# pashtari/factorizer

Measured on AMD Instinct MI355X. Metric: volumes/sec fwd+bwd, Swin Factorizer 128^3, higher is better.
Workload: dtype f32

## Files before the change

### factorizer_amd/csrc/conv3.hip

```cpp
#include "gemm_bx.h"

namespace fz {

template <typename AT>
struct Conv3ArgsT {
  const AT* x;
  const float* w;
  const float* bias;
  AT* y;
  int B, Cin, M, D, H, W;
  BlockPrologueArgs pro;
};

template <int MB, typename AT>
__global__ __launch_bounds__(256, 2) void conv3_fwd_kernel(Conv3ArgsT<AT> p) {
  extern __shared__ __attribute__((aligned(16))) float As[];
  const int lane = threadIdx.x & 63, wave = threadIdx.x >> 6;
  const int j = lane & 31, h = lane >> 5;
  const int64_t V = (int64_t)p.D * p.H * p.W;
  const int tiles_per_sample = (int)((V + 511) / 512);
  const int b = blockIdx.x / tiles_per_sample;
  const int64_t n0 = ((int64_t)(blockIdx.x % tiles_per_sample) * 4 + wave) * 128;
  const int m0 = blockIdx.y * 32 * MB;
  const int ncp = p.Cin / 2;
  const int nA = ncp * 27;

  for (int base = threadIdx.x; base < nA * MB * 64; base += blockDim.x * 8) {
    float tmp[8];
#pragma unroll
    for (int uu = 0; uu < 8; ++uu) {
      const int idx = base + uu * blockDim.x;
      const bool in = idx < nA * MB * 64;
      const int ii = in ? idx : 0;
      const int l = ii & 63, mb = (ii >> 6) % MB, a = ii / (64 * MB);
      const int m = m0 + mb * 32 + (l & 31);
      const int c = 2 * (a / 27) + (l >> 5), tap = a % 27;
      const int mc = m < p.M ? m : p.M - 1;
      const float wv = p.w[((int64_t)mc * p.Cin + c) * 27 + tap];
      tmp[uu] = (in && m < p.M) ? wv : 0.f;
    }
#pragma unroll
    for (int uu = 0; uu < 8; ++uu) {
      const int idx = base + uu * blockDim.x;
      if (idx < nA * MB * 64) As[idx] = tmp[uu];
    }
  }
  __syncthreads();

  const int64_t col = n0 + 4 * j;
  const bool col_ok = col < V;
  const int64_t cc = col_ok ? col : 0;
  const int w0 = (int)(cc % p.W);
  const int h0 = (int)((cc / p.W) % p.H);
  const int d0 = (int)(cc / ((int64_t)p.W * p.H));
  const bool lok = w0 > 0, rok = w0 + 4 < p.W;

  f32x16 acc[MB][4];
#pragma unroll
  for (int mb = 0; mb < MB; ++mb)
#pragma unroll
    for (int q = 0; q < 4; ++q)
#pragma unroll
      for (int r = 0; r < 16; ++r) acc[mb][q][r] = 0.f;

  for (int cp = 0; cp < ncp; ++cp) {
    const AT* plane = p.x + ((int64_t)b * p.Cin + 2 * cp + h) * V;
#pragma unroll
    for (int kd = 0; kd < 3; ++kd) {
#pragma unroll
      for (int kh = 0; kh < 3; ++kh) {
        const int zd = d0 + kd - 1, zh = h0 + kh - 1;
        const bool ok = col_ok && zd >= 0 && zd < p.D && zh >= 0 && zh < p.H;
        const int zdc = zd < 0 ? 0 : (zd >= p.D ? p.D - 1 : zd);
        const int zhc = zh < 0 ? 0 : (zh >= p.H ? p.H - 1 : zh);
        const AT* row = plane + ((int64_t)zdc * p.H + zhc) * p.W;
        const float4 t = ld4(row + w0);
        const float lf = aget(row + (lok ? w0 - 1 : w0));
        const float rt = aget(row + (rok ? w0 + 4 : w0));
        const float c0 = ok ? t.x : 0.f, c1 = ok ? t.y : 0.f, c2 = ok ? t.z : 0.f, c3 = ok ? t.w : 0.f;
        const float l0 = (ok && lok) ? lf : 0.f, r0 = (ok && rok) ? rt : 0.f;
        const float bv[3][4] = {{l0, c0, c1, c2}, {c0, c1, c2, c3}, {c1, c2, c3, r0}};
#pragma unroll
        for (int kw = 0; kw < 3; ++kw) {
          const int a = cp * 27 + (kd * 3 + kh) * 3 + kw;
#pragma unroll
          for (int mb = 0; mb < MB; ++mb) {
            const float av = As[(a * MB + mb) * 64 + lane];
#pragma unroll
            for (int q = 0; q < 4; ++q)
              acc[mb][q] = __builtin_amdgcn_mfma_f32_32x32x2f32(av, bv[kw][q], acc[mb][q], 0, 0, 0);
          }
        }
      }
    }
  }
  if (!col_ok) return;
#pragma unroll
  for (int mb = 0; mb < MB; ++mb)
#pragma unroll
    for (int r = 0; r < 16; ++r) {
      const int m = m0 + mb * 32 + (r & 3) + 8 * (r >> 2) + 4 * h;
      if (m >= p.M) continue;
      const float bs = p.bias ? p.bias[m] : 0.f;
      st4(p.y + ((int64_t)b * p.M + m) * V + col,
          make_float4(acc[mb][0][r] + bs, acc[mb][1][r] + bs, acc[mb][2][r] + bs, acc[mb][3][r] + bs));
    }
}

template <int MB, int CP, typename AT, bool PRO = false>
__global__ __launch_bounds__(256, 2) void conv3_fwd_bx_kernel(Conv3ArgsT<AT> p) {
  static_assert(!PRO || MB == 1, "the block prologue needs all 32 output channels in one row block");
  constexpr int NTA = BxTerms<AT>::A, NTB = bx_terms_b<AT>(BXPRO_NONE);
  constexpr int NS = CP * 27;
  constexpr int NG = (NS + 7) / 8;
  __shared__ __attribute__((aligned(16))) __bf16 As[NG * MB * NTA * 64 * 8];
  __shared__ float sBias[32 * MB];
  __shared__ __attribute__((aligned(16))) __bf16 Apro[PRO ? 2 * 3 * 64 * 8 : 8];
  __shared__ float twp[PRO ? 32 : 1];
  if constexpr (PRO) ln_inproj_stage(Apro, twp, p.pro, (int)threadIdx.x, 256);
  const int lane = threadIdx.x & 63, wave = threadIdx.x >> 6;
  const int j = lane & 31, h = lane >> 5;
  const int64_t V = (int64_t)p.D * p.H * p.W;
  const int tiles_per_sample = (int)((V + 511) / 512);
  const int b = blockIdx.x / tiles_per_sample;
  const int64_t n0 = ((int64_t)(blockIdx.x % tiles_per_sample) * 4 + wave) * 128;
  const int m0 = blockIdx.y * 32 * MB;
  const int Cin = 2 * CP;

  for (int idx = threadIdx.x; idx < NG * MB * 64; idx += 256) {
    const int l = idx & 63, mb = (idx >> 6) % MB, g = idx / (64 * MB);
    const int m = m0 + mb * 32 + (l & 31);
    const int mc = m < p.M ? m : p.M - 1;
    float wv[8];
#pragma unroll
    for (int e = 0; e < 8; ++e) {
      const int a = 8 * g + e;
      const int ac = a < NS ? a : NS - 1;
      const int c = 2 * (ac / 27) + (l >> 5), tap = ac % 27;
      const float t = p.w[((int64_t)mc * Cin + c) * 27 + tap];
      wv[e] = (a < NS && m < p.M) ? t : 0.f;
    }
    bx8 t3[NTA];
    bx_split<NTA>(wv, t3);
#pragma unroll
    for (int i = 0; i < NTA; ++i) *reinterpret_cast<bx8*>(&As[(((g * MB + mb) * NTA + i) * 64 + l) * 8]) = t3[i];
  }
  if (threadIdx.x < 32 * MB) {
    const int m = m0 + threadIdx.x;
    sBias[threadIdx.x] = (p.bias != nullptr && m < p.M) ? p.bias[m] : 0.f;
  }
  __syncthreads();

  const int64_t col = n0 + 4 * j;
  const bool col_ok = col < V;
  const int64_t cc = col_ok ? col : 0;
  const int w0 = (int)(cc % p.W);
  const int h0 = (int)((cc / p.W) % p.H);
  const int d0 = (int)(cc / ((int64_t)p.W * p.H));
  const bool lok = w0 > 0, rok = w0 + 4 < p.W;

  f32x16 acc[MB][4];
#pragma unroll
  for (int mb = 0; mb < MB; ++mb)
#pragma unroll
    for (int q = 0; q < 4; ++q)
#pragma unroll
      for (int r = 0; r < 16; ++r) acc[mb][q][r] = 0.f;

  float xg[4][8];
#pragma unroll
  for (int cp = 0; cp < CP; ++cp) {
    const AT* plane = p.x + ((int64_t)b * Cin + 2 * cp + h) * V;
#pragma unroll
    for (int kd = 0; kd < 3; ++kd) {
#pragma unroll
      for (int kh = 0; kh < 3; ++kh) {
        const int zd = d0 + kd - 1, zh = h0 + kh - 1;
        const bool ok = col_ok && zd >= 0 && zd < p.D && zh >= 0 && zh < p.H;
        const int zdc = zd < 0 ? 0 : (zd >= p.D ? p.D - 1 : zd);
        const int zhc = zh < 0 ? 0 : (zh >= p.H ? p.H - 1 : zh);
        const AT* row = plane + ((int64_t)zdc * p.H + zhc) * p.W;
        const float4 t = ld4(row + w0);
        const float lf = aget(row + (lok ? w0 - 1 : w0));
        const float rt = aget(row + (rok ? w0 + 4 : w0));
        const float c0 = ok ? t.x : 0.f, c1 = ok ? t.y : 0.f, c2 = ok ? t.z : 0.f, c3 = ok ? t.w : 0.f;
        const float l0 = (ok && lok) ? lf : 0.f, r0 = (ok && rok) ? rt : 0.f;
        const float bv[3][4] = {{l0, c0, c1, c2}, {c0, c1, c2, c3}, {c1, c2, c3, r0}};
#pragma unroll
        for (int kw = 0; kw < 3; ++kw) {
          const int a = cp * 27 + (kd * 3 + kh) * 3 + kw;
#pragma unroll
          for (int q = 0; q < 4; ++q) xg[q][a & 7] = bv[kw][q];
          if ((a & 7) == 7 || a == NS - 1) {
            const int g = a >> 3;
            if (a == NS - 1) {
#pragma unroll
              for (int e = (NS - 1) % 8 + 1; e < 8; ++e)
#pragma unroll
                for (int q = 0; q < 4; ++q) xg[q][e] = 0.f;
            }
            bx8 bop[4][NTB];
#pragma unroll
            for (int q = 0; q < 4; ++q) bx_split<NTB>(xg[q], bop[q]);
#pragma unroll
            for (int mb = 0; mb < MB; ++mb) {
              bx8 aop[NTA];
#pragma unroll
              for (int i = 0; i < NTA; ++i)
                aop[i] = *reinterpret_cast<const bx8*>(&As[(((g * MB + mb) * NTA + i) * 64 + lane) * 8]);
#pragma unroll
              for (int q = 0; q < 4; ++q) bx_mfma<NTA, NTB>(acc[mb][q], aop, bop[q]);
            }
          }
        }
      }
    }
  }
  if (!col_ok) return;
  float yv[PRO ? 4 : 1][16];
#pragma unroll
  for (int mb = 0; mb < MB; ++mb)
#pragma unroll
    for (int r = 0; r < 16; ++r) {
      const int rl = (r & 3) + 8 * (r >> 2) + 4 * h;
      const int m = m0 + mb * 32 + rl;
      const float bs = sBias[mb * 32 + rl];
      const float4 o = make_float4(acc[mb][0][r] + bs, acc[mb][1][r] + bs, acc[mb][2][r] + bs, acc[mb][3][r] + bs);
      if (m < p.M) st4(p.y + ((int64_t)b * p.M + m) * V + col, o);
      if constexpr (PRO) {
        constexpr bool R = sizeof(AT) == 2;
        yv[0][r] = R ? (float)(AT)o.x : o.x; yv[1][r] = R ? (float)(AT)o.y : o.y;
        yv[2][r] = R ? (float)(AT)o.z : o.z; yv[3][r] = R ? (float)(AT)o.w : o.w;
      }
    }
  if constexpr (PRO) {
    float mu[4], rs[4];
    f32x16 tacc[4];
    ln_inproj_tile<4>(yv, Apro, p.pro.ln_eps, lane, mu, rs, tacc);
    AT* tb = reinterpret_cast<AT*>(p.pro.t) + (int64_t)b * 32 * V + col;
#pragma unroll
    for (int r = 0; r < 16; ++r) {
      const int rl = (r & 3) + 8 * (r >> 2) + 4 * h;
      const float add = twp[rl];
      st4(tb + (int64_t)rl * V, make_float4(fmaxf(tacc[0][r] + add, 0.f), fmaxf(tacc[1][r] + add, 0.f), fmaxf(tacc[2][r] + add, 0.f),
                                            fmaxf(tacc[3][r] + add, 0.f)));
    }
    if (h == 0) {
      float* so = p.pro.stats + (int64_t)b * 2 * V + col;
      *reinterpret_cast<float4*>(so) = make_float4(mu[0], mu[1], mu[2], mu[3]);
      *reinterpret_cast<float4*>(so + V) = make_float4(rs[0], rs[1], rs[2], rs[3]);
    }
  }
}

template <typename AT>
struct Conv3WgradArgsT {
  const AT* gy;
  const AT* x;
  float* part;
  float* part_bias;
  int B, Cin, M, D, H, W;
  int tiles_per_unit;
};

constexpr int kXs = 44;

template <int KB, typename AT, bool BX = false>
__global__ __launch_bounds__(256) void conv3_wgrad_kernel(Conv3WgradArgsT<AT> a) {
  extern __shared__ __attribute__((aligned(16))) float lds[];
  const int lane = threadIdx.x & 63, wave = threadIdx.x >> 6;
  const int nrow = a.Cin * 9;
  const int per_wave = 32 * 36 + 36 * kXs;
  float* Pt = lds + wave * per_wave;
  float* Xs = Pt + 32 * 36;
  const int K = 27 * a.Cin;
  const int m0 = blockIdx.y * 32;
  const int64_t V = (int64_t)a.D * a.H * a.W;
  const int64_t tiles_per_sample = V / 32;
  const int64_t total = tiles_per_sample * a.B;
  const int64_t unit = (int64_t)blockIdx.x * 4 + wave;
  const int64_t t_begin = unit * a.tiles_per_unit, t_end = min(t_begin + a.tiles_per_unit, total);
  const int c = lane & 31, h = lane >> 5;

  int xoff[KB];
#pragma unroll
  for (int jb = 0; jb < KB; ++jb) {
    const int k = jb * 32 + c;
    const int kc = k < K ? k : 0;
    const int ci = kc / 27, tap = kc % 27;
    xoff[jb] = (ci * 9 + tap / 3) * kXs + 3 + (tap % 3);
  }
  f32x16 acc[KB];
#pragma unroll
  for (int jb = 0; jb < KB; ++jb)
#pragma unroll
    for (int r = 0; r < 16; ++r) acc[jb][r] = 0.f;
  float psum = 0.f;

  float4 pv[4], hv[5];
  float ev[2];
  int tb, td, th, tw;
  {
    const unsigned tps32 = (unsigned)tiles_per_sample;
    const unsigned t0 = (unsigned)__builtin_amdgcn_readfirstlane((int)t_begin);
    const unsigned rem = t0 % tps32, row = rem / (unsigned)(a.W / 32);
    tb = (int)(t0 / tps32);
    tw = (int)(rem % (unsigned)(a.W / 32)) * 32;
    th = (int)(row % (unsigned)a.H);
    td = (int)(row / (unsigned)a.H);
  }
  const unsigned bias = (unsigned)((a.H + 1) * a.W + 1);
  unsigned goff[4], xo[5], eo[2];
  unsigned xsafe[5], esafe[2];
  unsigned mask = 0;
  bool gvalid[4];
#pragma unroll
  for (int i = 0; i < 4; ++i) {
    const int m = m0 + (lane >> 3) + 8 * i;
    gvalid[i] = m < a.M;
    goff[i] = (unsigned)((m < a.M ? m : a.M - 1) * V + (lane & 7) * 4);
  }
  auto tap_bits = [&](int kd, int kh) { return (unsigned)((kd == 0) | ((kd == 2) << 1) | ((kh == 0) << 2) | ((kh == 2) << 3)); };
#pragma unroll
  for (int i = 0; i < 5; ++i) {
    const int q = lane + 64 * i;
    const int rr = min(q >> 3, nrow - 1), cq = q & 7;
    const int ci = rr / 9, kd = (rr % 9) / 3, kh = rr % 3;
    xo[i] = (unsigned)(ci * V + ((kd - 1) * a.H + (kh - 1)) * a.W + cq * 4 + (int64_t)bias);
    xsafe[i] = (unsigned)(ci * V + cq * 4 + (int64_t)bias);
    mask |= tap_bits(kd, kh) << (4 * i);
  }
#pragma unroll
  for (int i = 0; i < 2; ++i) {
    const int id = lane + 64 * i;
    const int rr = min(id >> 1, nrow - 1), side = id & 1;
    const int ci = rr / 9, kd = (rr % 9) / 3, kh = rr % 3;
    eo[i] = (unsigned)(ci * V + ((kd - 1) * a.H + (kh - 1)) * a.W + (side ? 32 : -1) + (int64_t)bias);
    esafe[i] = (unsigned)(ci * V + (int64_t)bias);
  }
  unsigned emask = 0, enever = 0;
#pragma unroll
  for (int i = 0; i < 2; ++i) {
    const int id = lane + 64 * i;
    const int rr = min(id >> 1, nrow - 1), side = id & 1;
    const int kd = (rr % 9) / 3, kh = rr % 3;
    emask |= (tap_bits(kd, kh) | (side ? 0x20u : 0x10u)) << (8 * i);
    enever |= ((id >> 1) < nrow ? 0u : 1u) << i;
  }
  unsigned xnever = 0;
#pragma unroll
  for (int i = 0; i < 5; ++i) xnever |= (((lane + 64 * i) >> 3) < nrow ? 0u : 1u) << i;
  auto issue = [&]() {
    const int b = tb, w0 = tw, h0 = th, d0 = td;
    const unsigned f4 = (unsigned)((d0 == 0) | ((d0 == a.D - 1) << 1) | ((h0 == 0) << 2) | ((h0 == a.H - 1) << 3));
    const unsigned f20 = f4 * 0x11111u;
    const unsigned fe = (f4 | ((w0 == 0) << 4) | ((w0 + 32 == a.W) << 5)) * 0x101u;
    const int64_t n0 = ((int64_t)d0 * a.H + h0) * a.W + w0;
    const AT* gbase = a.gy + (int64_t)b * a.M * V + n0;
    const AT* xbase = a.x + (int64_t)b * a.Cin * V + n0 - (int64_t)bias;
    tw += 32;
    if (tw == a.W) { tw = 0; if (++th == a.H) { th = 0; if (++td == a.D) { td = 0; ++tb; } } }
    const unsigned bad = mask & f20, ebad = emask & fe;
#pragma unroll
    for (int i = 0; i < 4; ++i) {
      const float4 v = ld4(gbase + goff[i]);
      pv[i] = gvalid[i] ? v : make_float4(0.f, 0.f, 0.f, 0.f);
    }
#pragma unroll
    for (int i = 0; i < 5; ++i) {
      const bool ok = ((bad >> (4 * i)) & 0xfu) == 0 && ((xnever >> i) & 1u) == 0;
      const float4 v = ld4(xbase + (ok ? xo[i] : xsafe[i]));
      hv[i] = ok ? v : make_float4(0.f, 0.f, 0.f, 0.f);
    }
#pragma unroll
    for (int i = 0; i < 2; ++i) {
      const bool ok = ((ebad >> (8 * i)) & 0x3fu) == 0 && ((enever >> i) & 1u) == 0;
      const float v = aget(xbase + (ok ? eo[i] : esafe[i]));
      ev[i] = ok ? v : 0.f;
    }
  };

  if (t_begin < t_end) issue();
  for (int64_t t = t_begin; t < t_end; ++t) {
#pragma unroll
    for (int i = 0; i < 4; ++i)
      *reinterpret_cast<float4*>(Pt + ((lane >> 3) + 8 * i) * 36 + (lane & 7) * 4) = pv[i];
#pragma unroll
    for (int i = 0; i < 5; ++i) {
      const int q = lane + 64 * i;
      if (q < 288) *reinterpret_cast<float4*>(Xs + (q >> 3) * kXs + 4 + (q & 7) * 4) = hv[i];
    }
#pragma unroll
    for (int i = 0; i < 2; ++i) {
      const int id = lane + 64 * i;
      if (id < 72) Xs[(id >> 1) * kXs + ((id & 1) ? 36 : 3)] = ev[i];
    }
    __builtin_amdgcn_fence(__ATOMIC_ACQ_REL, "wavefront");
    if (t + 1 < t_end) issue();
    if constexpr (BX) {
      constexpr int NTA = BxTerms<AT>::A;
      constexpr int NT = sizeof(AT) == 4 ? 3 : 1;
      (void)NTA;
#pragma unroll
      for (int g = 0; g < 2; ++g) {
        float a8[8];
        const float4 a0 = *reinterpret_cast<const float4*>(Pt + c * 36 + 16 * g + 8 * h);
        const float4 a1 = *reinterpret_cast<const float4*>(Pt + c * 36 + 16 * g + 8 * h + 4);
        a8[0] = a0.x; a8[1] = a0.y; a8[2] = a0.z; a8[3] = a0.w; a8[4] = a1.x; a8[5] = a1.y; a8[6] = a1.z; a8[7] = a1.w;
        psum += ((a8[0] + a8[1]) + (a8[2] + a8[3])) + ((a8[4] + a8[5]) + (a8[6] + a8[7]));
        bx8 aop[NT];
        bx_split<NT>(a8, aop);
#pragma unroll
        for (int jb = 0; jb < KB; ++jb) {
          float b8[8];
#pragma unroll
          for (int e = 0; e < 8; ++e) b8[e] = Xs[xoff[jb] + 16 * g + 8 * h + e];
          bx8 bop[NT];
          bx_split<NT>(b8, bop);
          bx_mfma<NT, NT>(acc[jb], aop, bop);
        }
      }
    } else {
#pragma unroll 4
    for (int s = 0; s < 16; ++s) {
      const float av = Pt[c * 36 + 2 * s + h];
      psum += av;
#pragma unroll
      for (int jb = 0; jb < KB; ++jb) {
        const float bv = Xs[xoff[jb] + 2 * s + h];
        acc[jb] = __builtin_amdgcn_mfma_f32_32x32x2f32(av, bv, acc[jb], 0, 0, 0);
      }
    }
    }
    __builtin_amdgcn_fence(__ATOMIC_ACQ_REL, "wavefront");
  }

  __syncthreads();
  float* red = lds;
#pragma unroll
  for (int jb = 0; jb < KB; ++jb) {
#pragma unroll
    for (int r = 0; r < 16; ++r) {
      const int row = (r & 3) + 8 * (r >> 2) + 4 * h;
      red[wave * 1024 + row * 32 + c] = acc[jb][r];
    }
    __syncthreads();
    for (int e = threadIdx.x; e < 1024; e += 256) {
      const float sres = (red[e] + red[1024 + e]) + (red[2048 + e] + red[3072 + e]);
      const int m = m0 + (e >> 5), k = jb * 32 + (e & 31);
      if (m < a.M && k < K) a.part[((int64_t)blockIdx.x * a.M + m) * K + k] = sres;
    }
    __syncthreads();
  }
  {
    const float sres = psum + __shfl_xor(psum, 32, 64);
    if (h == 0) red[wave * 32 + c] = sres;
    __syncthreads();
    if (threadIdx.x < 32) {
      const int m = m0 + threadIdx.x;
      if (m < a.M)
        a.part_bias[(int64_t)blockIdx.x * a.M + m] =
            (red[threadIdx.x] + red[32 + threadIdx.x]) + (red[64 + threadIdx.x] + red[96 + threadIdx.x]);
    }
  }
}

}

using namespace fz;

template <typename AT>
static int conv3_fwd_launch(const void* x, const float* w, const float* bias, void* y, int B, int Cin, int M, int D,
                            int H, int W, int products, const fz_block_prologue* pro, fz_stream_t stream) {
  Conv3ArgsT<AT> p{(const AT*)x, w, bias, (AT*)y, B, Cin, M, D, H, W, BlockPrologueArgs{}};
  if (pro) {
    if (!(Cin == 4 && M == 32 && products_split(products)))
      return fail(FZ_E_UNSUPPORTED, "fz_conv3_fwd2: the block prologue needs C_in = 4, 32 output channels, split-bf16 products (fz_conv3_prologue_supported)");
    p.pro = BlockPrologueArgs{pro->ln_g, pro->ln_b, pro->ln_eps, pro->w, pro->t, pro->stats};
  }
  const int64_t V = (int64_t)D * H * W;
  const int mblocks = (M + 31) / 32;
  const int MB = mblocks >= 2 ? 2 : 1;
  const size_t lds = (size_t)(Cin / 2) * 27 * MB * 64 * sizeof(float);
  if (lds > 65536) return fail(FZ_E_UNSUPPORTED, "fz_conv3_fwd: C_in too large for the stem kernel");
  dim3 grid((unsigned)(((V + 511) / 512) * B), (unsigned)((mblocks + MB - 1) / MB)), block(256);
  hipStream_t st = (hipStream_t)stream;
  if (Cin == 4 && products_split(products)) {
    if (MB == 2) hipLaunchKernelGGL((conv3_fwd_bx_kernel<2, 2, AT>), grid, block, 0, st, p);
    else if (pro) hipLaunchKernelGGL((conv3_fwd_bx_kernel<1, 2, AT, true>), grid, block, 0, st, p);
    else hipLaunchKernelGGL((conv3_fwd_bx_kernel<1, 2, AT>), grid, block, 0, st, p);
    FZ_LAUNCH_CHECK();
    return FZ_OK;
  }
  if (MB == 2) hipLaunchKernelGGL((conv3_fwd_kernel<2, AT>), grid, block, lds, st, p);
  else hipLaunchKernelGGL((conv3_fwd_kernel<1, AT>), grid, block, lds, st, p);
  FZ_LAUNCH_CHECK();
  return FZ_OK;
}

extern "C" int fz_conv3_prologue_supported(int Cin, int M, int W, int products) {
  return (Cin == 4 && M == 32 && W >= 4 && (W & 3) == 0 && products_split(products)) ? 1 : 0;
}

extern "C" int fz_conv3_fwd2(const void* x, const float* w, const float* bias, void* y, int B, int Cin, int M, int D,
                             int H, int W, int act_dtype, int products, const fz_block_prologue* pro, fz_stream_t stream) {
  if (!x || !w || !y) return fail(FZ_E_ARG, "fz_conv3_fwd: null pointer");
  if (pro && (!pro->ln_g || !pro->ln_b || !pro->w || !pro->t || !pro->stats)) return fail(FZ_E_ARG, "fz_conv3_fwd2: incomplete block prologue");
  if (B < 0 || Cin < 2 || (Cin & 1) || M < 1 || D < 1 || H < 1 || W < 4 || (W & 3))
    return fail(FZ_E_UNSUPPORTED, "fz_conv3_fwd: needs even C_in and W % 4 == 0");
  if (B == 0) return FZ_OK;
  if (act_dtype == FZ_STORE_F32) return conv3_fwd_launch<float>(x, w, bias, y, B, Cin, M, D, H, W, products, pro, stream);
  if (act_dtype == FZ_STORE_BF16) return conv3_fwd_launch<bf16>(x, w, bias, y, B, Cin, M, D, H, W, products, pro, stream);
  return fail(FZ_E_ARG, "fz_conv3_fwd: bad act_dtype");
}

extern "C" int fz_conv3_fwd(const void* x, const float* w, const float* bias, void* y, int B, int Cin, int M, int D,
                            int H, int W, int act_dtype, int products, fz_stream_t stream) {
  return fz_conv3_fwd2(x, w, bias, y, B, Cin, M, D, H, W, act_dtype, products, nullptr, stream);
}

static int conv3_units(int64_t total_tiles, int* tiles_per_unit) {
  int64_t units_target = 4096;
  int64_t tpu = (total_tiles + units_target - 1) / units_target;
  if (tpu < 1) tpu = 1;
  *tiles_per_unit = (int)tpu;
  const int64_t units = (total_tiles + tpu - 1) / tpu;
  return (int)((units + 3) / 4);
}

extern "C" int fz_conv3_wgrad_chunks(int B, int D, int H, int W) {
  int tpu;
  return conv3_units(((int64_t)D * H * W / 32) * B, &tpu);
}

template <typename AT>
static int conv3_wgrad_launch(const void* gy, const void* x, float* part, float* part_bias, int B, int Cin,
                              int M, int D, int H, int W, int products, fz_stream_t stream) {
  Conv3WgradArgsT<AT> a{(const AT*)gy, (const AT*)x, part, part_bias, B, Cin, M, D, H, W, 1};
  const int nchunk = conv3_units(((int64_t)D * H * W / 32) * B, &a.tiles_per_unit);
  const size_t lds = (size_t)4 * (32 * 36 + 36 * kXs) * sizeof(float);
  const size_t lds_red = 4096 * sizeof(float);
  dim3 grid(nchunk, (M + 31) / 32), block(256);
  if (products_split(products))
    hipLaunchKernelGGL((conv3_wgrad_kernel<4, AT, true>), grid, block, lds > lds_red ? lds : lds_red, (hipStream_t)stream, a);
  else
    hipLaunchKernelGGL((conv3_wgrad_kernel<4, AT, false>), grid, block, lds > lds_red ? lds : lds_red, (hipStream_t)stream, a);
  FZ_LAUNCH_CHECK();
  return FZ_OK;
}

extern "C" int fz_conv3_wgrad_partials(const void* gy, const void* x, float* part, float* part_bias, int B, int Cin,
                                       int M, int D, int H, int W, int act_dtype, int products, fz_stream_t stream) {
  if (!gy || !x || !part || !part_bias) return fail(FZ_E_ARG, "fz_conv3_wgrad: null pointer");
  if (B < 1 || Cin < 1 || M < 1 || (W % 32) || 27 * Cin > 128 || Cin * 9 > 36)
    return fail(FZ_E_UNSUPPORTED, "fz_conv3_wgrad: needs W % 32 == 0 and C_in <= 4");
  {
    const int64_t V = (int64_t)D * H * W;
    if ((V / 32) * B >= ((int64_t)1 << 31) || (int64_t)(M < 32 ? 32 : M) * V >= ((int64_t)1 << 32) ||
        (int64_t)Cin * V + (int64_t)(H + 1) * W + 64 >= ((int64_t)1 << 32))
      return fail(FZ_E_UNSUPPORTED, "fz_conv3_wgrad: volume too large for the kernel's 32-bit offsets");
  }
  if (act_dtype == FZ_STORE_F32) return conv3_wgrad_launch<float>(gy, x, part, part_bias, B, Cin, M, D, H, W, products, stream);
  if (act_dtype == FZ_STORE_BF16) return conv3_wgrad_launch<bf16>(gy, x, part, part_bias, B, Cin, M, D, H, W, products, stream);
  return fail(FZ_E_ARG, "fz_conv3_wgrad: bad act_dtype");
}
```

Baseline: 130.9.

## Pre-split bf16 operands once in conv3 fwd and wgrad, remap wgrad blocks per XCD

In the stem conv forward kernel, the row values are now split into bf16 terms once per (kd,kh) and packed as bf16 pairs, instead of being re-split per 8-element group. Address math moves to 32-bit offsets with boundary flag masks, and out-of-range columns stay in the loop with guarded stores. In wgrad, when the multi-term bf16 path is in use, the input tile is pre-split into bf16 levels stored in LDS and read back with alignbit shifts, avoiding repeated per-jb splitting. Blocks are also remapped so contiguous units land on the same XCD. This adds a 32-bit volume limit check and more LDS per wave.

Measured after the change: 130.9. Within noise of the previous version (-0.0%).

```diff
diff --git a/factorizer_amd/csrc/conv3.hip b/factorizer_amd/csrc/conv3.hip
--- a/factorizer_amd/csrc/conv3.hip
+++ b/factorizer_amd/csrc/conv3.hip
@@ -1,6 +1,8 @@
 #include "gemm_bx.h"
 
 namespace fz {
+
+typedef unsigned u32x4 __attribute__((ext_vector_type(4)));
 
 template <typename AT>
 struct Conv3ArgsT {
@@ -153,11 +155,17 @@
 
   const int64_t col = n0 + 4 * j;
   const bool col_ok = col < V;
-  const int64_t cc = col_ok ? col : 0;
-  const int w0 = (int)(cc % p.W);
-  const int h0 = (int)((cc / p.W) % p.H);
-  const int d0 = (int)(cc / ((int64_t)p.W * p.H));
+  const unsigned cc = col_ok ? (unsigned)col : 0u;
+  const unsigned rowi = cc / (unsigned)p.W;
+  const int w0 = (int)(cc % (unsigned)p.W);
+  const int h0 = (int)(rowi % (unsigned)p.H);
+  const int d0 = (int)(rowi / (unsigned)p.H);
   const bool lok = w0 > 0, rok = w0 + 4 < p.W;
+  const unsigned flags = (unsigned)((d0 == 0) | ((d0 == p.D - 1) << 1) | ((h0 == 0) << 2) | ((h0 == p.H - 1) << 3) | ((col_ok ? 0 : 1) << 4));
+  const unsigned Vu = (unsigned)V, HW = (unsigned)p.H * (unsigned)p.W, Wu = (unsigned)p.W;
+  const AT* xb = p.x + (int64_t)b * Cin * V;
+  const unsigned lo_c = (unsigned)h * Vu + cc;
+  const unsigned lo_l = lok ? lo_c - 1u : lo_c, lo_r = rok ? lo_c + 4u : lo_c;
 
   f32x16 acc[MB][4];
 #pragma unroll
@@ -167,41 +175,69 @@
 #pragma unroll
       for (int r = 0; r < 16; ++r) acc[mb][q][r] = 0.f;
 
-  float xg[4][8];
+  unsigned bw[4][NTB][4];
+  float pend[4][NTB];
 #pragma unroll
   for (int cp = 0; cp < CP; ++cp) {
-    const AT* plane = p.x + ((int64_t)b * Cin + 2 * cp + h) * V;
+    const unsigned cbase = (unsigned)(2 * cp) * Vu;
 #pragma unroll
     for (int kd = 0; kd < 3; ++kd) {
 #pragma unroll
       for (int kh = 0; kh < 3; ++kh) {
-        const int zd = d0 + kd - 1, zh = h0 + kh - 1;
-        const bool ok = col_ok && zd >= 0 && zd < p.D && zh >= 0 && zh < p.H;
-        const int zdc = zd < 0 ? 0 : (zd >= p.D ? p.D - 1 : zd);
-        const int zhc = zh < 0 ? 0 : (zh >= p.H ? p.H - 1 : zh);
-        const AT* row = plane + ((int64_t)zdc * p.H + zhc) * p.W;
-        const float4 t = ld4(row + w0);
-        const float lf = aget(row + (lok ? w0 - 1 : w0));
-        const float rt = aget(row + (rok ? w0 + 4 : w0));
-        const float c0 = ok ? t.x : 0.f, c1 = ok ? t.y : 0.f, c2 = ok ? t.z : 0.f, c3 = ok ? t.w : 0.f;
-        const float l0 = (ok && lok) ? lf : 0.f, r0 = (ok && rok) ? rt : 0.f;
-        const float bv[3][4] = {{l0, c0, c1, c2}, {c0, c1, c2, c3}, {c1, c2, c3, r0}};
+        constexpr unsigned kColBit = 0x10u;
+        const unsigned tb = (unsigned)((kd == 0) | ((kd == 2) << 1) | ((kh == 0) << 2) | ((kh == 2) << 3)) | kColBit;
+        const bool ok = (flags & tb) == 0;
+        const unsigned goff = ok ? cbase + (unsigned)(kd - 1) * HW + (unsigned)(kh - 1) * Wu : cbase;
+        const float4 t = ld4(xb + (lo_c + goff));
+        const float lf = aget(xb + (lo_l + goff));
+        const float rt = aget(xb + (lo_r + goff));
+        float rv[NTB][6];
+        rv[0][0] = (ok && lok) ? lf : 0.f; rv[0][1] = ok ? t.x : 0.f; rv[0][2] = ok ? t.y : 0.f;
+        rv[0][3] = ok ? t.z : 0.f; rv[0][4] = ok ? t.w : 0.f; rv[0][5] = (ok && rok) ? rt : 0.f;
+#pragma unroll
+        for (int l = 1; l < NTB; ++l)
+#pragma unroll
+          for (int i = 0; i < 6; i += 2) {
+            const fx2 v = {rv[l - 1][i], rv[l - 1][i + 1]};
+            const fx2 d = v - __builtin_convertvector(__builtin_convertvector(v, bx2), fx2);
+            rv[l][i] = d[0]; rv[l][i + 1] = d[1];
+          }
 #pragma unroll
         for (int kw = 0; kw < 3; ++kw) {
           const int a = cp * 27 + (kd * 3 + kh) * 3 + kw;
 #pragma unroll
-          for (int q = 0; q < 4; ++q) xg[q][a & 7] = bv[kw][q];
+          for (int q = 0; q < 4; ++q)
+#pragma unroll
+            for (int l = 0; l < NTB; ++l) {
+              if ((a & 1) == 0) {
+                pend[q][l] = rv[l][kw + q];
+                if (a == NS - 1) {
+                  const fx2 v = {pend[q][l], 0.f};
+                  bw[q][l][(a & 7) >> 1] = __builtin_bit_cast(unsigned, __builtin_convertvector(v, bx2));
+                }
+              } else {
+                const fx2 v = {pend[q][l], rv[l][kw + q]};
+                bw[q][l][(a & 7) >> 1] = __builtin_bit_cast(unsigned, __builtin_convertvector(v, bx2));
+              }
+            }
           if ((a & 7) == 7 || a == NS - 1) {
             const int g = a >> 3;
             if (a == NS - 1) {
 #pragma unroll
-              for (int e = (NS - 1) % 8 + 1; e < 8; ++e)
-#pragma unroll
-                for (int q = 0; q < 4; ++q) xg[q][e] = 0.f;
+              for (int e = ((NS - 1) % 8) / 2 + 1; e < 4; ++e)
+#pragma unroll
+                for (int q = 0; q < 4; ++q)
+#pragma unroll
+                  for (int l = 0; l < NTB; ++l) bw[q][l][e] = 0u;
             }
             bx8 bop[4][NTB];
 #pragma unroll
-            for (int q = 0; q < 4; ++q) bx_split<NTB>(xg[q], bop[q]);
+            for (int q = 0; q < 4; ++q)
+#pragma unroll
+              for (int l = 0; l < NTB; ++l) {
+                const u32x4 o = {bw[q][l][0], bw[q][l][1], bw[q][l][2], bw[q][l][3]};
+                bop[q][l] = __builtin_bit_cast(bx8, o);
+              }
 #pragma unroll
             for (int mb = 0; mb < MB; ++mb) {
               bx8 aop[NTA];
@@ -216,7 +252,7 @@
       }
     }
   }
-  if (!col_ok) return;
+  if constexpr (!PRO) { if (!col_ok) return; }
   float yv[PRO ? 4 : 1][16];
 #pragma unroll
   for (int mb = 0; mb < MB; ++mb)
@@ -226,7 +262,7 @@
       const int m = m0 + mb * 32 + rl;
       const float bs = sBias[mb * 32 + rl];
       const float4 o = make_float4(acc[mb][0][r] + bs, acc[mb][1][r] + bs, acc[mb][2][r] + bs, acc[mb][3][r] + bs);
-      if (m < p.M) st4(p.y + ((int64_t)b * p.M + m) * V + col, o);
+      if (m < p.M && col_ok) st4(p.y + ((int64_t)b * p.M + m) * V + col, o);
       if constexpr (PRO) {
         constexpr bool R = sizeof(AT) == 2;
         yv[0][r] = R ? (float)(AT)o.x : o.x; yv[1][r] = R ? (float)(AT)o.y : o.y;
@@ -242,10 +278,11 @@
     for (int r = 0; r < 16; ++r) {
       const int rl = (r & 3) + 8 * (r >> 2) + 4 * h;
       const float add = twp[rl];
-      st4(tb + (int64_t)rl * V, make_float4(fmaxf(tacc[0][r] + add, 0.f), fmaxf(tacc[1][r] + add, 0.f), fmaxf(tacc[2][r] + add, 0.f),
-                                            fmaxf(tacc[3][r] + add, 0.f)));
-    }
-    if (h == 0) {
+      if (col_ok)
+        st4(tb + (int64_t)rl * V, make_float4(fmaxf(tacc[0][r] + add, 0.f), fmaxf(tacc[1][r] + add, 0.f), fmaxf(tacc[2][r] + add, 0.f),
+                                              fmaxf(tacc[3][r] + add, 0.f)));
+    }
+    if (h == 0 && col_ok) {
       float* so = p.pro.stats + (int64_t)b * 2 * V + col;
       *reinterpret_cast<float4*>(so) = make_float4(mu[0], mu[1], mu[2], mu[3]);
       *reinterpret_cast<float4*>(so + V) = make_float4(rs[0], rs[1], rs[2], rs[3]);
@@ -265,30 +302,71 @@
 
 constexpr int kXs = 44;
 
+constexpr int kXl = 18;
+constexpr int kXr = 3 * kXl;
+constexpr int conv3_wgrad_per_wave(bool lv) { return 32 * 36 + 36 * (lv ? kXr : kXs); }
+constexpr bool conv3_wgrad_levels(int nt) { return nt == 3; }
+template <typename AT> struct Conv3WgradTerms { static constexpr int N = sizeof(AT) == 4 ? 3 : 1; };
+
+template <int NT>
+__device__ __forceinline__ void bx_split2(float x0, float x1, unsigned (&t)[NT]) {
+  fx2 v = {x0, x1};
+  const bx2 a = __builtin_convertvector(v, bx2);
+  t[0] = __builtin_bit_cast(unsigned, a);
+  if constexpr (NT >= 2) {
+    v = v - __builtin_convertvector(a, fx2);
+    const bx2 b = __builtin_convertvector(v, bx2);
+    t[1] = __builtin_bit_cast(unsigned, b);
+    if constexpr (NT >= 3) {
+      v = v - __builtin_convertvector(b, fx2);
+      const bx2 c = __builtin_convertvector(v, bx2);
+      t[2] = __builtin_bit_cast(unsigned, c);
+    }
+  }
+}
+
+__device__ __forceinline__ int conv3_wgrad_logical_block() {
+  const int nb = (int)gridDim.x, bid = (int)blockIdx.x;
+  if (nb < 16) return bid;
+  const int q = nb / 8, r = nb % 8, xcd = bid % 8, i = bid / 8;
+  return (xcd < r ? xcd * (q + 1) : r * (q + 1) + (xcd - r) * q) + i;
+}
+
 template <int KB, typename AT, bool BX = false>
 __global__ __launch_bounds__(256) void conv3_wgrad_kernel(Conv3WgradArgsT<AT> a) {
   extern __shared__ __attribute__((aligned(16))) float lds[];
   const int lane = threadIdx.x & 63, wave = threadIdx.x >> 6;
   const int nrow = a.Cin * 9;
-  const int per_wave = 32 * 36 + 36 * kXs;
-  float* Pt = lds + wave * per_wave;
-  float* Xs = Pt + 32 * 36;
+  constexpr int NT = Conv3WgradTerms<AT>::N;
+  constexpr bool LV = BX && conv3_wgrad_levels(NT);
+  constexpr int XR = kXr;
+  const int per_wave = conv3_wgrad_per_wave(LV);
+  float* Pt = lds + wave * per_wave + (LV ? 36 * XR : 0);
+  float* Xs = lds + wave * per_wave + (LV ? 0 : 32 * 36);
+  unsigned* Xl = reinterpret_cast<unsigned*>(Xs);
+  const int lb = LV ? conv3_wgrad_logical_block() : (int)blockIdx.x;
   const int K = 27 * a.Cin;
   const int m0 = blockIdx.y * 32;
   const int64_t V = (int64_t)a.D * a.H * a.W;
   const int64_t tiles_per_sample = V / 32;
   const int64_t total = tiles_per_sample * a.B;
-  const int64_t unit = (int64_t)blockIdx.x * 4 + wave;
+  const int64_t unit = (int64_t)lb * 4 + wave;
   const int64_t t_begin = unit * a.tiles_per_unit, t_end = min(t_begin + a.tiles_per_unit, total);
   const int c = lane & 31, h = lane >> 5;
 
   int xoff[KB];
+  unsigned xsh = 0;
 #pragma unroll
   for (int jb = 0; jb < KB; ++jb) {
     const int k = jb * 32 + c;
     const int kc = k < K ? k : 0;
     const int ci = kc / 27, tap = kc % 27;
-    xoff[jb] = (ci * 9 + tap / 3) * kXs + 3 + (tap % 3);
+    if constexpr (LV) {
+      xoff[jb] = (ci * 9 + tap / 3) * XR + (tap % 3 ? 1 : 0);
+      xsh |= (tap % 3 != 1 ? 1u : 0u) << jb;
+    } else {
+      xoff[jb] = (ci * 9 + tap / 3) * kXs + 3 + (tap % 3);
+    }
   }
   f32x16 acc[KB];
 #pragma unroll
@@ -385,6 +463,31 @@
 #pragma unroll
     for (int i = 0; i < 4; ++i)
       *reinterpret_cast<float4*>(Pt + ((lane >> 3) + 8 * i) * 36 + (lane & 7) * 4) = pv[i];
+    if constexpr (LV) {
+#pragma unroll
+      for (int i = 0; i < 5; ++i) {
+        const int q = lane + 64 * i;
+        unsigned lo[NT], hi[NT];
+        bx_split2<NT>(hv[i].x, hv[i].y, lo);
+        bx_split2<NT>(hv[i].z, hv[i].w, hi);
+        if (q < 288) {
+          unsigned* d = Xl + (q >> 3) * XR + 1 + (q & 7) * 2;
+#pragma unroll
+          for (int l = 0; l < NT; ++l) { d[l * kXl] = lo[l]; d[l * kXl + 1] = hi[l]; }
+        }
+      }
+#pragma unroll
+      for (int i = 0; i < 2; ++i) {
+        const int id = lane + 64 * i;
+        unsigned lv[NT];
+        bx_split2<NT>(ev[i], 0.f, lv);
+        if (id < 72) {
+          unsigned short* d = reinterpret_cast<unsigned short*>(Xl + (id >> 1) * XR) + ((id & 1) ? 34 : 1);
+#pragma unroll
+          for (int l = 0; l < NT; ++l) d[l * kXl * 2] = (unsigned short)lv[l];
+        }
+      }
+    } else {
 #pragma unroll
     for (int i = 0; i < 5; ++i) {
       const int q = lane + 64 * i;
@@ -395,12 +498,10 @@
       const int id = lane + 64 * i;
       if (id < 72) Xs[(id >> 1) * kXs + ((id & 1) ? 36 : 3)] = ev[i];
     }
+    }
     __builtin_amdgcn_fence(__ATOMIC_ACQ_REL, "wavefront");
     if (t + 1 < t_end) issue();
     if constexpr (BX) {
-      constexpr int NTA = BxTerms<AT>::A;
-      constexpr int NT = sizeof(AT) == 4 ? 3 : 1;
-      (void)NTA;
 #pragma unroll
       for (int g = 0; g < 2; ++g) {
         float a8[8];
@@ -412,11 +513,25 @@
         bx_split<NT>(a8, aop);
 #pragma unroll
         for (int jb = 0; jb < KB; ++jb) {
-          float b8[8];
-#pragma unroll
-          for (int e = 0; e < 8; ++e) b8[e] = Xs[xoff[jb] + 16 * g + 8 * h + e];
           bx8 bop[NT];
-          bx_split<NT>(b8, bop);
+          if constexpr (!LV) {
+            float b8[8];
+#pragma unroll
+            for (int e = 0; e < 8; ++e) b8[e] = Xs[xoff[jb] + 16 * g + 8 * h + e];
+            bx_split<NT>(b8, bop);
+          }
+          const unsigned* src = Xl + xoff[jb] + 4 * (2 * g + h);
+          const unsigned sh = ((xsh >> jb) & 1u) * 16u;
+#pragma unroll
+          for (int l = 0; l < (LV ? NT : 0); ++l) {
+            unsigned dw[5];
+#pragma unroll
+            for (int e = 0; e < 5; ++e) dw[e] = src[l * kXl + e];
+            u32x4 o;
+#pragma unroll
+            for (int e = 0; e < 4; ++e) o[e] = __builtin_amdgcn_alignbit(dw[e + 1], dw[e], sh);
+            bop[l] = __builtin_bit_cast(bx8, o);
+          }
           bx_mfma<NT, NT>(acc[jb], aop, bop);
         }
       }
@@ -448,7 +563,7 @@
     for (int e = threadIdx.x; e < 1024; e += 256) {
       const float sres = (red[e] + red[1024 + e]) + (red[2048 + e] + red[3072 + e]);
       const int m = m0 + (e >> 5), k = jb * 32 + (e & 31);
-      if (m < a.M && k < K) a.part[((int64_t)blockIdx.x * a.M + m) * K + k] = sres;
+      if (m < a.M && k < K) a.part[((int64_t)lb * a.M + m) * K + k] = sres;
     }
     __syncthreads();
   }
@@ -459,7 +574,7 @@
     if (threadIdx.x < 32) {
       const int m = m0 + threadIdx.x;
       if (m < a.M)
-        a.part_bias[(int64_t)blockIdx.x * a.M + m] =
+        a.part_bias[(int64_t)lb * a.M + m] =
             (red[threadIdx.x] + red[32 + threadIdx.x]) + (red[64 + threadIdx.x] + red[96 + threadIdx.x]);
     }
   }
@@ -486,6 +601,8 @@
   dim3 grid((unsigned)(((V + 511) / 512) * B), (unsigned)((mblocks + MB - 1) / MB)), block(256);
   hipStream_t st = (hipStream_t)stream;
   if (Cin == 4 && products_split(products)) {
+    if ((int64_t)Cin * V >= ((int64_t)1 << 32))
+      return fail(FZ_E_UNSUPPORTED, "fz_conv3_fwd: volume too large for the kernel's 32-bit offsets");
     if (MB == 2) hipLaunchKernelGGL((conv3_fwd_bx_kernel<2, 2, AT>), grid, block, 0, st, p);
     else if (pro) hipLaunchKernelGGL((conv3_fwd_bx_kernel<1, 2, AT, true>), grid, block, 0, st, p);
     else hipLaunchKernelGGL((conv3_fwd_bx_kernel<1, 2, AT>), grid, block, 0, st, p);
@@ -538,7 +655,7 @@
                               int M, int D, int H, int W, int products, fz_stream_t stream) {
   Conv3WgradArgsT<AT> a{(const AT*)gy, (const AT*)x, part, part_bias, B, Cin, M, D, H, W, 1};
   const int nchunk = conv3_units(((int64_t)D * H * W / 32) * B, &a.tiles_per_unit);
-  const size_t lds = (size_t)4 * (32 * 36 + 36 * kXs) * sizeof(float);
+  const size_t lds = (size_t)4 * conv3_wgrad_per_wave(products_split(products) && conv3_wgrad_levels(Conv3WgradTerms<AT>::N)) * sizeof(float);
   const size_t lds_red = 4096 * sizeof(float);
   dim3 grid(nchunk, (M + 31) / 32), block(256);
   if (products_split(products))
```
